# 17ai/eventql

Measured on AMD Instinct MI355X. Metric: rows/sec scanned+aggregated, 1e9-row 4-col GROUP BY, higher is better.
Workload: dtype u64/f64; 1 GPU; config3; query=k, sum(v), count(1), sum(b) WHERE a>30000 AND b<30000 GROUP BY k, rows_per_gpu=1000000000, columns=4, encodings=UINT64_PLAIN/FLOAT_IEEE754, groups=1000, partitions=1, merge=none, groups_hint=given, float_sums=fast

## Files before the change

### eventql_amd/csrc/codegen.h

```cpp
#pragma once
#include <string>
#include <vector>
#include "cstable_format.h"
#include "plan_ir.h"

namespace evql {

struct ColAccess {
  enum Mode { PLAIN64 = 0, PLAIN32 = 1, BITPACKED = 2, SOA = 3, NARROW = 4, NARROW_F32 = 5 };
  std::string name;
  uint32_t stype = EVQL_T_NIL;
  Mode mode = PLAIN64;
  uint32_t bits = 0;
  bool has_tags = false;
  bool bool_normalize = false;
  bool from_uint_to_float = false;
  bool string_hash = false;
  bool string_bytes = false;
  bool packed = false;
  bool dict_code = false;
  int layout_index = -1;
};

struct StateWord {
// ... 2 lines not shown

struct AggPlan {
  uint32_t fn = EVQL_AGG_NONE;
  ExprPtr arg;
  int first_word = 0;
  int nwords = 0;
  int distinct_index = -1;
  int exact_index = -1;
  bool narrow_arg = false;
};

static const int kMaxExactSums = 4;

static const int kMaxDistinct = 4;

static const int kMaxLits = 32;

static const uint64_t kZoneRows = 2048;
static const int kMaxZoneConjuncts = 4;

struct ZoneConjunct {
  int col = -1;
  uint32_t op = 0;
  uint64_t lit = 0;
};

enum KeyMode {
  KEY_NONE = 0,
  KEY_EXACT = 1,
  KEY_HASHED = 2
};

struct KernelPlan {
  std::vector<ColAccess> cols;
  ExprPtr where;
  std::vector<ExprPtr> group;
  std::vector<AggPlan> aggs;
  std::vector<StateWord> states;
  KeyMode key_mode = KEY_NONE;
  bool need_first_row = false;
  bool has_row_filter = false;
  int n_distinct = 0;
  int n_exact = 0;
  bool has_ident2() const { return key_mode == KEY_HASHED; }
  int first_row_word() const { return 1 + (has_ident2() ? 1 : 0); }
  int words_per_slot() const { return state_word_base() + int(states.size()); }
  int state_word_base() const { return first_row_word() + (need_first_row ? 1 : 0); }
  int block = 256;
  int unroll = 4;
  int lds_slots = 0;
  int lane_cache = 1;
  bool prefetch = false;
  bool prefetch_allowed = false;
  bool partitioned = false;
  int part_bits = 12;
  bool part_fused = false;
  bool narrow_ident = false;
  bool narrow_first_row = false;
  bool where_rows_kernel = false;
  bool bare_scan = false;
  std::vector<ExprPtr> scan_out;
  std::vector<bool> scan_out_nullable;
  std::vector<uint64_t> lit_pool;
  std::vector<ZoneConjunct> zone_conjuncts;
  int tile_rows() const { return block * 2 * unroll; }
};

void choose_launch_shape(KernelPlan* kp, uint64_t hint);
uint64_t lds_table_max_slots(const KernelPlan& kp);
extern const uint64_t kPartitionAboveSlots;
bool partitioned_path_possible(const KernelPlan& kp);

bool expr_prints_zero_check(const ExprPtr& e);

std::string generate_kernel_source(KernelPlan* kp);
int partition_tuple_u32_words(const KernelPlan& kp);

const char* device_library_source();

}
```

### eventql_amd/csrc/codegen_kernels.inc

```

namespace {

struct UpdWord {
  int word;
  int op;
  int tslot = -1;
  const char* constant = nullptr;
  bool narrow = false;
  int toff = -1;
};

struct Gen {
  const KernelPlan& kp;
  std::ostringstream s;
  const int NC, NW, S, W, SB;
  const bool grouped;
  std::vector<UpdWord> updw;

  explicit Gen(const KernelPlan& p)
      : kp(p), NC(int(p.cols.size())), NW(int(p.states.size())), S(p.lds_slots),
        W(p.words_per_slot()), SB(p.state_word_base()), grouped(p.key_mode != KEY_NONE) {
    for (const auto& a : kp.aggs) {
      switch (a.fn) {
        case EVQL_AGG_COUNT:
// ... 91 lines not shown
    char b[96];
    snprintf(b, sizeof(b), "A.gtab[(u64) %s * EVQL_WORDS + %d]", slot.c_str(), w);
    return b;
  }

  void prologue() {
    s << "// generated by eventql_amd codegen\n";
    s << "#define EVQL_BLOCK " << kp.block << "\n";
    s << "#define EVQL_UNROLL " << kp.unroll << "\n";
    s << "#define EVQL_TILE_ROWS " << kp.tile_rows() << "\n";
    s << "#define EVQL_LDS_SLOTS " << S << "\n";
    s << "#define EVQL_LSTRIDE " << (S + 2) << "\n";
    s << "#define EVQL_WORDS " << W << "\n";
    s << "#define EVQL_NSTATE " << NW << "\n";
    s << "#define EVQL_NUPD " << (U() > 0 ? U() : 1) << "\n";
    s << "#define EVQL_LCACHE " << kp.lane_cache << "\n";
    s << "#define EVQL_TUPLE_U32 " << tuple_u32 << "\n";
    s << "#define EVQL_TIF " << (tuple_u32 <= 10 ? 4 : 2) << "\n\n";
    s << "struct EvqlRowOut {\n  bool live;\n  bool knull;\n  u64 ident;\n  u64 ident2;\n"
         "  u64 ub[EVQL_NUPD];\n  bool uc[EVQL_NUPD];\n};\n\n";
  }

  template <typename Body>
  size_t row_function(size_t lit_base, Body body) {
    const std::string before = s.str();
    s.str("");
    Emitter em;
    em.lit_base = lit_base;
    em.pool = &pool;
    em.cols = &kp.cols;
    body(em);
    const std::string fn = s.str();
    s.str("");
    s << before;
    if (em.uses_strfn && !strfn_emitted) {
      s << strfn_library_source();
      strfn_emitted = true;
    }
    for (size_t i = 0; i < em.string_literals.size(); ++i) {
      const std::string& l = em.string_literals[i];
      s << "__device__ const u8 evql_slit" << (lit_base + i) << "[" << (l.empty() ? 1 : l.size())
        << "] = {";
      for (size_t k = 0; k < l.size(); ++k) s << (k ? "," : "") << unsigned((unsigned char) l[k]);
      if (l.empty()) s << "0";
      s << "};\n";
    }
    s << fn;
    return em.string_literals.size();
  }

  bool strfn_emitted = false;
  size_t n_literals = 0;
  std::vector<uint64_t> pool;
  void eval_row() {
    n_literals = row_function(0, [&](Emitter& em) { eval_row_body(em); });
  }

  void col_decls() {
    for (int i = 0; i < NC; ++i) {
      const ColAccess& c = kp.cols[i];
      s << "  const " << ctype(c.stype) << " c" << i << " = ";
      if (c.stype == EVQL_T_FLOAT64) {
        s << (c.from_uint_to_float ? "(double) r" : "evql_as_f64(r") << i
          << (c.from_uint_to_float ? "" : ")") << ";\n";
      } else if (c.stype == EVQL_T_BOOL) {
        s << "(r" << i << " != 0);\n";
      } else if (c.stype == EVQL_T_INT64) {
        s << "(i64) r" << i << ";\n";
      } else {
        s << "r" << i << ";\n";
      }
      s << "  (void) c" << i << "; (void) g" << i << ";\n";
    }
  }

  void eval_row_body(Emitter& em) {
    s << "__device__ __forceinline__ void evql_eval_row(const EvqlArgs& A, const u64 row, "
         "const bool valid";
    for (int i = 0; i < NC; ++i) s << ", const u64 r" << i << ", const u32 g" << i;
    s << ", EvqlRowOut& o) {\n";
    s << "  bool live = valid;\n";
    if (kp.has_row_filter) {
      s << "  live = live && evql_row_filter(A.row_filter, A.row_filter_len, row);\n";
    }
    col_decls();
    em.ind = "    ";
    if (kp.where) {
      s << "  if (live) {\n";
      Val p = em.emit(kp.where);
      s << em.o.str();
      em.o.str("");
      s << "    live = " << p.v << ";\n  }\n";
    }
    s << "  o.live = live;\n  o.knull = false;\n  o.ident = 0;\n  o.ident2 = 0;\n";
    for (int i = 0; i < U(); ++i) {
      s << "  o.ub[" << i << "] = evql_op_identity<" << op_name(updw[i].op) << ">(); o.uc[" << i
        << "] = false;\n";
    }
    s << "  if (live) {\n";
    if (kp.key_mode == KEY_EXACT) {
      Val k = em.emit(kp.group[0]);
      s << em.o.str();
      em.o.str("");
      s << "    o.ident = " << Emitter::as_bits(k) << ";\n";
      s << "    o.knull = (" << k.g << " & 1u) != 0;\n";
    } else if (kp.key_mode == KEY_HASHED) {
      s << "    u64 ident = EVQL_IDENT_SEED1, ident2 = EVQL_IDENT_SEED2;\n";
      for (const auto& g : kp.group) {
        Val k = em.emit(g);
        s << em.o.str();
        em.o.str("");
        s << "    evql_ident_add(ident, ident2, " << Emitter::as_bits(k) << ", " << k.g << ");\n";
      }
      s << "    o.ident = evql_ident_word(ident);\n";
      s << "    o.ident2 = evql_ident_word(ident2);\n";
    }
    int ui = 0;
    auto push = [&](const std::string& bits, const std::string& cond) {
      if (cond.empty()) {
        s << "    o.ub[" << ui << "] = " << bits << "; o.uc[" << ui << "] = true;\n";
      } else {
        s << "    o.uc[" << ui << "] = " << cond << ";\n";
        s << "    if (o.uc[" << ui << "]) o.ub[" << ui << "] = " << bits << ";\n";
      }
      ++ui;
    };
    for (const auto& a : kp.aggs) {
      Val v{"0", "0u", EVQL_T_NIL};
      if (a.arg) {
        v = em.emit(a.arg);
        s << em.o.str();
        em.o.str("");
      }
      const std::string notnull = "((" + v.g + " & 1u) == 0)";
      switch (a.fn) {
        case EVQL_AGG_COUNT:
          push("1ull", "");
          break;
        case EVQL_AGG_SUM_UINT64:
        case EVQL_AGG_SUM_INT64:
          push(Emitter::as_bits(v), "");
          break;
        case EVQL_AGG_SUM_FLOAT64:
          if (a.exact_index >= 0) {
            s << "    u64 fxh" << a.exact_index << ", fxl" << a.exact_index << ";\n";
            s << "    evql_fix(A, " << a.exact_index << ", " << v.v << ", fxh" << a.exact_index
              << ", fxl" << a.exact_index << ");\n";
            push("fxh" + std::to_string(a.exact_index), "");
            push("fxl" + std::to_string(a.exact_index), "");
          } else {
            push(Emitter::as_bits(v), "");
          }
          break;
        case EVQL_AGG_COUNT_DISTINCT_UINT64: {
          const char* flags = kp.key_mode == KEY_HASHED ? "o.ident2"
                              : (kp.key_mode == KEY_EXACT ? "(o.knull ? 1ull : 0ull)" : "0ull");
          char b[64];
          snprintf(b, sizeof(b), "evql_pairset_insert(A, %d, o.ident, ", a.distinct_index);
          push(std::string(b) + Emitter::as_bits(v) + ", " + flags + ", " +
                   (kp.key_mode == KEY_HASHED ? "false" : "true") + ")",
               "");
          break;
        }
        case EVQL_AGG_MEAN_UINT64:
        case EVQL_AGG_MEAN_INT64:
        case EVQL_AGG_MEAN_FLOAT64: {
          std::string d = a.fn == EVQL_AGG_MEAN_FLOAT64 ? v.v : "((double) " + v.v + ")";
          push("evql_f64_bits(" + d + ")", notnull);
          push("1ull", notnull);
          break;
        }
        default: {
          const bool is_f = a.fn == EVQL_AGG_MIN_FLOAT64 || a.fn == EVQL_AGG_MAX_FLOAT64;
          const std::string ok = is_f ? "(" + notnull + " && (" + v.v + " == " + v.v + "))" : notnull;
          push(Emitter::as_bits(v), ok);
          push("1ull", ok);
        }
      }
    }
    s << "  }\n}\n\n";
  }

  void tile_loads(const char* ind, const std::vector<bool>* only = nullptr) {
    for (int i = 0; i < NC; ++i) {
      if (only && !(*only)[i]) continue;
      s << ind << "u64 x" << i << "[EVQL_UNROLL][2]; u32 y" << i << "[EVQL_UNROLL][2];\n";
    }
    s << "#pragma unroll\n" << ind << "for (int u = 0; u < EVQL_UNROLL; ++u) {\n";
    s << ind << "  const u64 r = base + ((u64) (u * EVQL_BLOCK) + tid) * 2;\n";
    for (int i = 0; i < NC; ++i) {
      if (only && !(*only)[i]) continue;
      const ColAccess& c = kp.cols[i];
      switch (c.mode) {
        case ColAccess::PLAIN64:
          s << ind << "  evql_plain64_x2(A.col[" << i << "].base, A.col[" << i << "].pages, r, x" << i << "[u][0], x"
            << i << "[u][1]);\n";
          break;
        case ColAccess::PLAIN32:
          s << ind << "  evql_plain32_x2(A.col[" << i << "].base, A.col[" << i << "].pages, r, x" << i << "[u][0], x"
            << i << "[u][1]);\n";
          break;
        case ColAccess::BITPACKED:
          s << ind << "  evql_bitpacked_x2<" << c.bits << ">(A.col[" << i << "].base, A.col[" << i << "].pages, r, x"
            << i << "[u][0], x" << i << "[u][1]);\n";
          break;
        case ColAccess::NARROW:
          s << ind << "  evql_bitpacked_x2<" << c.bits << ">(A.col[" << i << "].base, r, x" << i
            << "[u][0], x" << i << "[u][1]);\n";
          break;
        case ColAccess::NARROW_F32:
          s << ind << "  evql_f32_x2(A.col[" << i << "].base, r, x" << i << "[u][0], x" << i
            << "[u][1]);\n";
          break;
        case ColAccess::SOA:
          s << ind << "  evql_soa_x2(A.col[" << i << "].soa, r, x" << i << "[u][0], x" << i
            << "[u][1]);\n";
          break;
      }
      if (c.has_tags) {
        s << ind << "  { const unsigned short tt = *reinterpret_cast<const unsigned short*>(A.col["
          << i << "].tags + r); y" << i << "[u][0] = tt & 0xffu; y" << i << "[u][1] = tt >> 8; }\n";
      } else {
        s << ind << "  y" << i << "[u][0] = 0; y" << i << "[u][1] = 0;\n";
      }
    }
    s << ind << "}\n";
  }

  bool prunes() const { return !kp.zone_conjuncts.empty(); }
  bool zone_test = false;
  template <typename Loop>
  void tile_loop_twice(const char* ind, Loop emit_loop) {
    zone_test = false;
// ... 69 lines not shown
      s << ind << "u32 " << name << i << "[EVQL_UNROLL][" << raw_words(kp.cols[i]) << "]"
        << (zero ? " = {}" : "") << ";\n";
    }
  }
  void raw_tile_loads(const char* ind) {
    s << "#pragma unroll\n" << ind << "for (int u = 0; u < EVQL_UNROLL; ++u) {\n";
    s << ind << "  const u64 r = lbase + ((u64) (u * EVQL_BLOCK) + tid) * 2;\n";
    for (int i = 0; i < NC; ++i) {
      const ColAccess& c = kp.cols[i];
      const int hi = raw_words(c) - 1;
      if (c.mode == ColAccess::NARROW_F32) {
        s << ind << "  evql_f32_x2(A.col[" << i << "].base, r, n" << i << "[u][0], n" << i << "[u][" << hi
          << "]);\n";
      } else {
        s << ind << "  evql_bitpacked_x2<" << c.bits << ">(A.col[" << i << "].base, r, n" << i << "[u][0], n"
          << i << "[u][" << hi << "]);\n";
      }
    }
    s << ind << "}\n";
  }
  void raw_step_decode(const char* ind) {
    s << ind << "asm(\"\" : ";
    bool first = true;
    for (int i = 0; i < NC; ++i) {
      for (int w = 0; w < raw_words(kp.cols[i]); ++w) {
        s << (first ? "" : ", ") << "\"+v\"(c" << i << "[u][" << w << "])";
        first = false;
      }
    }
    s << ");\n";
    for (int i = 0; i < NC; ++i) {
      const ColAccess& c = kp.cols[i];
      const int hi = raw_words(c) - 1;
      s << ind << "u64 x" << i << "s[2]; ";
      if (c.mode == ColAccess::NARROW_F32) {
        s << "evql_f32_dec(c" << i << "[u][0], c" << i << "[u][" << hi << "], x" << i << "s[0], x" << i
          << "s[1]);\n";
      } else {
        s << "evql_narrow_dec<" << c.bits << ">(c" << i << "[u][0], c" << i << "[u][" << hi << "], x" << i
          << "s[0], x" << i << "s[1]);\n";
      }
    }
  }
  void raw_tile_copy(const char* ind) {
    s << "#pragma unroll\n" << ind << "for (int u = 0; u < EVQL_UNROLL; ++u) {\n" << ind << " ";
    for (int i = 0; i < NC; ++i) {
      for (int w = 0; w < raw_words(kp.cols[i]); ++w) {
        s << " c" << i << "[u][" << w << "] = n" << i << "[u][" << w << "];";
      }
    }
    s << "\n" << ind << "}\n";
  }

  bool probe_ahead() const { return grouped && S > 0 && !kp.has_ident2(); }
  void scan_step(const std::string& ind, bool step_local) {
    const char* in = ind.c_str();
    if (probe_ahead()) {
      s << in << "EvqlRowOut o0, o1;\n";
      for (int j = 0; j < 2; ++j) eval_call(in, j, nullptr, j ? "o1" : "o0", step_local);
      for (int j = 0; j < 2; ++j) {
        s << in << "const u64 k" << j << " = evql_lds_peek(&lds[(u32) o" << j
          << ".ident & (EVQL_LDS_SLOTS - 1)]);\n";
      }
      for (int j = 0; j < 2; ++j) {
        s << in << "evql_update(A, lds, acc, bypass, r + " << j << ", o" << j << ", k" << j << ");\n";
      }
    } else {
      s << in << "EvqlRowOut o;\n";
      for (int j = 0; j < 2; ++j) {
        eval_call(in, j, nullptr, "o", step_local);
        s << in << "evql_update(A, lds, acc, bypass, r + " << j << ", o);\n";
      }
    }
  }
  void prefetch_tile_loop() {
    s << "  u32 tile_no = 0;  // tiles evaluated\n";
    raw_tile_decls("  ", "c", false);
    s << "  bool have = false;\n  u64 tc = 0;\n";
    s << "  for (u64 t = blockIdx.x; have || t < A.ntiles; t += gridDim.x) {\n";
    s << "    const bool more = t < A.ntiles;\n";
    s << "    const u64 tl = more ? t : tc;\n";
    s << "    u32 st = 0;\n";
    s << "    if ((tile_no & 15u) == 0) st = __hip_atomic_load(&A.status[0], __ATOMIC_RELAXED, "
         "__HIP_MEMORY_SCOPE_AGENT);\n";
    s << "    const u64 lbase = (A.tile0 + tl) * (u64) EVQL_TILE_ROWS;\n";
    raw_tile_decls("    ", "n", false);
    raw_tile_loads("    ");
    s << "    __builtin_amdgcn_sched_barrier(0);\n";
    s << "    if (have) {\n";
    s << "      const bool bypass = evql_lds_peek32(reinterpret_cast<const u32*>(&lds[EVQL_WORDS * "
         "EVQL_LSTRIDE])) >= 4u * EVQL_BLOCK;\n";
    s << "      const u64 base = (A.tile0 + tc) * (u64) EVQL_TILE_ROWS;\n";
    tile_window("      ");
    s << "#pragma unroll\n      for (int u = 0; u < EVQL_UNROLL; ++u) {\n";
    s << "        const u64 r = base + ((u64) (u * EVQL_BLOCK) + tid) * 2;\n";
    raw_step_decode("        ");
    scan_step("        ", true);
    s << "      }\n      ++tile_no;\n    }\n";
    s << "    __builtin_amdgcn_sched_barrier(0);\n";
    raw_tile_copy("    ");
    s << "    asm volatile(\"\" : \"+v\"(st)";
    for (int i = 0; i < NC; ++i) {
      for (int w = 0; w < raw_words(kp.cols[i]); ++w) s << ", \"+v\"(c" << i << "[EVQL_UNROLL - 1][" << w << "])";
    }
    s << ");\n";
    s << "    tc = tl;\n    have = more;\n";
    s << "    if (__builtin_amdgcn_readfirstlane(st) & EVQL_ST_TABLE_FULL) break;\n";
    s << "  }\n";
  }
  void scan_kernel() {
    const char* ctr = kp.prefetch ? "u32" : "u64";
    s << "struct EvqlAcc {\n  " << ctr << " passed;\n  " << ctr << " spilled;\n";
    if (!grouped) s << "  u64 w[" << (NW > 0 ? NW : 1) << "];\n";
    if (!grouped && kp.need_first_row) s << "  u64 first;\n";
    if (grouped && S > 0) {
      s << "  int cs[EVQL_LCACHE];\n  u64 cfirst[EVQL_LCACHE];\n  u64 cw[EVQL_LCACHE][EVQL_NUPD];\n"
           "  u32 cv;\n";
    }
    s << "};\n\n";
    if (grouped && S > 0) {
      s << "template <int J>\n";
      s << "__device__ __forceinline__ void evql_flush_entry(u64* lds, EvqlAcc& acc) {\n";
      s << "  const int cs = acc.cs[J];\n";
      if (kp.need_first_row) {
        s << "  evql_atomic<EVQL_OP_MIN_U64>(&" << lds_word(kp.first_row_word(), "cs") << ", acc.cfirst[J]);\n";
        s << "  acc.cfirst[J] = 0xFFFFFFFFFFFFFFFFull;\n";
      }
      for (int i = 0; i < U(); ++i) {
        s << "  evql_atomic<" << op_name(updw[i].op) << ">(&" << lds_word(SB + updw[i].word, "cs")
          << ", acc.cw[J][" << i << "]);\n";
        s << "  acc.cw[J][" << i << "] = evql_op_identity<" << op_name(updw[i].op) << ">();\n";
      }
      s << "}\n";
      s << "__device__ __forceinline__ void evql_flush_private(u64* lds, EvqlAcc& acc) {\n";
      for (int j = 0; j < kp.lane_cache; ++j) {
        s << "  if (acc.cs[" << j << "] >= 0) { evql_flush_entry<" << j << ">(lds, acc); acc.cs[" << j
          << "] = -1; }\n";
      }
      s << "}\n\n";
    }

    s << "__device__ __forceinline__ void evql_update(const EvqlArgs& A, u64* lds, EvqlAcc& acc,\n"
         "                                            const bool bypass, const u64 row, "
         "const EvqlRowOut& o"
      << (probe_ahead() ? ", const u64 slot0" : "") << ") {\n";
    s << "  acc.passed += o.live ? 1 : 0;\n";
    if (!grouped) {
      if (kp.need_first_row) s << "  if (o.live && row < acc.first) acc.first = row;\n";
      for (int i = 0; i < U(); ++i) {
        s << "  if (o.uc[" << i << "]) acc.w[" << updw[i].word << "] = evql_combine<"
          << op_name(updw[i].op) << ">(acc.w[" << updw[i].word << "], o.ub[" << i << "]);\n";
      }
      s << "}\n\n";
    } else {
      auto updates = [&](bool global, const char* slot, const char* ind) {
        if (kp.need_first_row) {
          s << ind << "evql_atomic<EVQL_OP_MIN_U64>(&"
            << (global ? gtab_word(kp.first_row_word(), slot) : lds_word(kp.first_row_word(), slot))
            << ", row);\n";
        }
        for (int i = 0; i < U(); ++i) {
// ... 89 lines not shown
    }

    if (grouped && S > 0) {
      s << "__device__ __forceinline__ void evql_lds_init(u64* lds) {\n";
      s << "  if (threadIdx.x == 0) lds[EVQL_WORDS * EVQL_LSTRIDE] = 0;\n";
      s << "  for (u32 i = threadIdx.x; i < EVQL_LSTRIDE; i += blockDim.x) {\n";
      s << "    lds[i] = EVQL_EMPTY;\n";
      if (kp.has_ident2()) s << "    lds[1 * EVQL_LSTRIDE + i] = EVQL_EMPTY;\n";
      if (kp.need_first_row) {
        s << "    " << lds_word(kp.first_row_word(), "i") << " = 0xFFFFFFFFFFFFFFFFull;\n";
      }
      for (int w = 0; w < NW; ++w) {
        s << "    " << lds_word(SB + w, "i") << " = evql_op_identity<" << op_name(kp.states[w].op)
          << ">();\n";
      }
      s << "  }\n}\n\n";
      s << "template <bool EXCL>\n";
      s << "__device__ __forceinline__ void evql_lds_flush(const EvqlArgs& A, u64* lds) {\n";
      s << "  const bool excl = EXCL && evql_lds_peek32(reinterpret_cast<const u32*>(&lds[EVQL_WORDS * EVQL_LSTRIDE])) "
           "== 0;\n";
      s << "  for (u32 s = threadIdx.x; s < EVQL_LSTRIDE; s += blockDim.x) {\n";
      s << "    const u64 k = lds[s];\n    if (k == EVQL_EMPTY) continue;\n";
      s << "    i64 gs;\n";
      s << "    if (s == EVQL_LDS_SLOTS) gs = (i64) A.gcap;\n";
      s << "    else if (s == EVQL_LDS_SLOTS + 1) gs = (i64) A.gcap + 1;\n";
      if (kp.has_ident2()) {
        s << "    else gs = evql_gtab_find2(A.gtab, EVQL_WORDS, A.gcap, k, lds[EVQL_LSTRIDE + s], "
             "evql_mix64(k));\n";
      } else {
        s << "    else gs = evql_gtab_find(A.gtab, EVQL_WORDS, A.gcap, k, evql_mix64(k));\n";
      }
      s << "    if (gs < 0) { atomicOr(&A.status[0], EVQL_ST_TABLE_FULL); continue; }\n";
      s << "    if (s >= EVQL_LDS_SLOTS) A.gtab[(u64) gs * EVQL_WORDS] = 0;\n";
      s << "    if (excl) {\n";
      if (kp.need_first_row) {
        s << "      " << gtab_word(kp.first_row_word(), "gs") << " = " << lds_word(kp.first_row_word(), "s")
          << ";\n";
      }
      for (int w = 0; w < NW; ++w) {
        s << "      " << gtab_word(SB + w, "gs") << " = " << lds_word(SB + w, "s") << ";\n";
      }
      s << "      continue;\n    }\n";
      if (kp.need_first_row) {
        s << "    evql_atomic<EVQL_OP_MIN_U64>(&" << gtab_word(kp.first_row_word(), "gs") << ", "
          << lds_word(kp.first_row_word(), "s") << ");\n";
      }
      for (int w = 0; w < NW; ++w) {
        s << "    evql_atomic<" << op_name(kp.states[w].op) << ">(&" << gtab_word(SB + w, "gs") << ", "
          << lds_word(SB + w, "s") << ");\n";
      }
      s << "  }\n}\n\n";
    }

    s << "extern \"C\" __global__ void __launch_bounds__(EVQL_BLOCK) evql_scan_agg(const EvqlArgs A) {\n";
    s << "  const u32 tid = threadIdx.x;\n";
    if (grouped && S > 0) {
      s << "  __shared__ u64 lds[EVQL_WORDS * EVQL_LSTRIDE + 1];\n";
      s << "  evql_lds_init(lds);\n  __syncthreads();\n";
    } else {
      s << "  u64* lds = nullptr;\n";
    }
    s << "  EvqlAcc acc;\n  acc.passed = 0;\n  acc.spilled = 0;\n";
    if (grouped && S > 0) {
      s << "  acc.cv = 0;\n";
      for (int j = 0; j < kp.lane_cache; ++j) {
        s << "  acc.cs[" << j << "] = -1;\n  acc.cfirst[" << j << "] = 0xFFFFFFFFFFFFFFFFull;\n";
        for (int i = 0; i < U(); ++i) {
          s << "  acc.cw[" << j << "][" << i << "] = evql_op_identity<" << op_name(updw[i].op) << ">();\n";
        }
      }
    }
    if (!grouped) {
      for (int w = 0; w < NW; ++w) {
        s << "  acc.w[" << w << "] = evql_op_identity<" << op_name(kp.states[w].op) << ">();\n";
      }
      if (kp.need_first_row) s << "  acc.first = 0xFFFFFFFFFFFFFFFFull;\n";
    }
    zone_skip_decl("  ");
    window32 = grouped;
    tile_loop_twice("  ", [&] {
    if (kp.prefetch && !zone_test && grouped && S > 0) {
      prefetch_tile_loop();
      return;
    }
    s << "  u32 tile_no = 0;\n";
    s << "  for (u64 t = blockIdx.x; t < A.ntiles; t += gridDim.x, ++tile_no) {\n";
    zone_skip("    ", "");
    if (grouped) {
      s << "    if ((tile_no & 15u) == 0 && (__hip_atomic_load(&A.status[0], __ATOMIC_RELAXED, "
           "__HIP_MEMORY_SCOPE_AGENT) & EVQL_ST_TABLE_FULL)) break;\n";
    }
    if (grouped && S > 0) {
      s << "    const bool bypass = evql_lds_peek32(reinterpret_cast<const u32*>(&lds[EVQL_WORDS * EVQL_LSTRIDE])) "
           ">= 4u * EVQL_BLOCK;\n";
    } else {
      s << "    const bool bypass = false;\n";
    }
    s << "    const u64 base = (A.tile0 + t) * (u64) EVQL_TILE_ROWS;\n";
    tile_window("    ");
    tile_loads("    ");
    s << "#pragma unroll\n    for (int u = 0; u < EVQL_UNROLL; ++u) {\n";
    s << "      const u64 r = base + ((u64) (u * EVQL_BLOCK) + tid) * 2;\n";
    scan_step("      ", false);
    s << "    }\n  }\n";
    });
    window32 = true;

    zone_skip_flush("  ");
    s << "  {\n    const u64 p = evql_wave_reduce<EVQL_OP_ADD_U64>(" << (kp.prefetch ? "(u64) " : "") << "acc.passed);\n";
    s << "    if ((tid & 63u) == 0 && p) atomicAdd(&A.counters[0], p);\n";
// ... 610 lines not shown
```

### eventql_amd/csrc/evql_device.h

```cpp
#ifndef EVQL_DEVICE_H
#define EVQL_DEVICE_H

typedef unsigned long long u64;
typedef long long i64;
typedef unsigned int u32;
typedef unsigned char u8;

#define EVQL_EMPTY 0xFFFFFFFFFFFFFFFFull
#define EVQL_MAX_COLS 16
#define EVQL_MAX_LITS 32
#define EVQL_WAVE 64

#define EVQL_ST_DIV_BY_ZERO 1u
#define EVQL_ST_TABLE_FULL 2u
#define EVQL_ST_MOD_BY_ZERO 4u

struct EvqlColArg {
  const u64* pages;
  const u64* soa;
  const u8* tags;
  u64 npages;
  const u64* strpos;
  const u8* base;
};
// ... 308 lines not shown
#define EVQL_OP_MIN_F64 6
#define EVQL_OP_MAX_F64 7

template <int OP>
__device__ __forceinline__ u64 evql_op_identity() {
  switch (OP) {
    case EVQL_OP_MIN_U64: return 0xFFFFFFFFFFFFFFFFull;
    case EVQL_OP_MAX_U64: return 0ull;
    case EVQL_OP_MIN_I64: return 0x7FFFFFFFFFFFFFFFull;
    case EVQL_OP_MAX_I64: return 0x8000000000000000ull;
    case EVQL_OP_MIN_F64: return 0x7FF0000000000000ull;
    case EVQL_OP_MAX_F64: return 0xFFF0000000000000ull;
    default: return 0ull;
  }
}

template <int OP>
__device__ __forceinline__ u64 evql_combine(u64 a, u64 b) {
  switch (OP) {
    case EVQL_OP_ADD_U64: return a + b;
    case EVQL_OP_ADD_F64: return evql_f64_bits(evql_as_f64(a) + evql_as_f64(b));
    case EVQL_OP_MIN_U64: return a < b ? a : b;
    case EVQL_OP_MAX_U64: return a > b ? a : b;
    case EVQL_OP_MIN_I64: return (i64) a < (i64) b ? a : b;
    case EVQL_OP_MAX_I64: return (i64) a > (i64) b ? a : b;
    case EVQL_OP_MIN_F64: return evql_as_f64(b) < evql_as_f64(a) ? b : a;
    case EVQL_OP_MAX_F64: return evql_as_f64(b) > evql_as_f64(a) ? b : a;
  }
  return a;
}

template <int OP>
__device__ __forceinline__ void evql_atomic(u64* p, u64 v) {
  switch (OP) {
    case EVQL_OP_ADD_U64: atomicAdd(p, v); break;
    case EVQL_OP_ADD_F64: unsafeAtomicAdd(reinterpret_cast<double*>(p), evql_as_f64(v)); break;
    case EVQL_OP_MIN_U64: atomicMin(p, v); break;
    case EVQL_OP_MAX_U64: atomicMax(p, v); break;
    case EVQL_OP_MIN_I64: atomicMin(reinterpret_cast<i64*>(p), (i64) v); break;
    case EVQL_OP_MAX_I64: atomicMax(reinterpret_cast<i64*>(p), (i64) v); break;
    case EVQL_OP_MIN_F64: unsafeAtomicMin(reinterpret_cast<double*>(p), evql_as_f64(v)); break;
    case EVQL_OP_MAX_F64: unsafeAtomicMax(reinterpret_cast<double*>(p), evql_as_f64(v)); break;
  }
}


__device__ __forceinline__ u64 evql_lds_peek(const u64* p) {
  return __hip_atomic_load(p, __ATOMIC_RELAXED, __HIP_MEMORY_SCOPE_WORKGROUP);
}
__device__ __forceinline__ u32 evql_lds_peek32(const u32* p) {
  return __hip_atomic_load(p, __ATOMIC_RELAXED, __HIP_MEMORY_SCOPE_WORKGROUP);
}

template <int MAXP>
__device__ __forceinline__ int evql_lds_find_from(u64* keys, u32 mask, u64 ident, u32 h, u64 cur) {
  u32 s = (u32) ident & mask;
  {
    if (cur == ident) return (int) s;
    if (cur == EVQL_EMPTY) {
      u64 old = atomicCAS(&keys[s], EVQL_EMPTY, ident);
      if (old == EVQL_EMPTY || old == ident) return (int) s;
    }
  }
  s = h & mask;
#pragma unroll 1
  for (int probe = 0; probe < MAXP; ++probe) {
    u64 cur = evql_lds_peek(&keys[s]);
    if (cur == ident) return (int) s;
    if (cur == EVQL_EMPTY) {
      u64 old = atomicCAS(&keys[s], EVQL_EMPTY, ident);
      if (old == EVQL_EMPTY || old == ident) return (int) s;
    }
    s = (s + 1) & mask;
  }
  return -1;
}
template <int MAXP>
__device__ __forceinline__ int evql_lds_find(u64* keys, u32 mask, u64 ident, u32 h) {
  return evql_lds_find_from<MAXP>(keys, mask, ident, h, evql_lds_peek(&keys[(u32) ident & mask]));
}

#define EVQL_GTAB_MAX_PROBE 128
__device__ __forceinline__ i64 evql_gtab_find(u64* tab, u32 W, u64 cap, u64 ident, u64 h) {
  const u64 mask = cap - 1;
  u64 s = h & mask;
  const u64 maxp = cap < EVQL_GTAB_MAX_PROBE ? cap : EVQL_GTAB_MAX_PROBE;
#pragma unroll 1
  for (u64 probe = 0; probe < maxp; ++probe) {
    u64* key = tab + s * W;
    u64 cur = __hip_atomic_load(key, __ATOMIC_RELAXED, __HIP_MEMORY_SCOPE_AGENT);
    if (cur == ident) return (i64) s;
    if (cur == EVQL_EMPTY) {
      u64 old = atomicCAS(key, EVQL_EMPTY, ident);
      if (old == EVQL_EMPTY || old == ident) return (i64) s;
    }
    s = (s + 1) & mask;
  }
  return -1;
}

template <int MAXP>
__device__ __forceinline__ int evql_lds_find2(u64* keys, u64* keys2, u32 mask, u64 ident,
                                              u64 ident2, u32 h) {
  u32 s = (u32) ident & mask;
#pragma unroll 1
  for (int probe = 0; probe <= MAXP; ++probe) {
// ... 84 lines not shown
```

### eventql_amd/csrc/planner.cc

```cpp
#include <cstdlib>
#include <cstring>
#include "runtime.h"

namespace evql {

namespace {

ExprPtr inline_inputs(const ExprPtr& e, const std::vector<ExprPtr>& sub, std::string* err) {
  if (!e) return e;
  if (e->kind == Expr::INPUT) {
    if (e->input >= sub.size()) {
      *err = "invalid input index";
      return e;
    }
    return sub[e->input];
  }
  auto c = std::make_shared<Expr>(*e);
  for (auto& a : c->args) a = inline_inputs(a, sub, err);
  return c;
}

bool has_agg_get(const ExprPtr& e) {
  if (!e) return false;
  if (e->kind == Expr::AGG_GET) return true;
// ... 184 lines not shown
    const ExprPtr &c = e->args[k], &l = e->args[1 - k];
    if (c->kind == Expr::INPUT && l->kind == Expr::LITERAL && !l->lit_tag && unsigned_type(l->type)) ci = k;
  }
  if (ci < 0) return;
  const ExprPtr& c = e->args[ci];
  if (c->input >= cols.size() || !unsigned_type(c->type)) return;
  const ColAccess& ca = cols[c->input];
  if (ca.stype != c->type || ca.layout_index < 0) return;
  if (ca.from_uint_to_float || ca.bool_normalize || ca.string_hash || ca.has_tags) return;
  if (!zone_column_qualifies(layout.columns[ca.layout_index])) return;
  ZoneConjunct z;
  z.col = int(c->input);
  z.lit = e->args[1 - ci]->lit_bits;
  switch (e->family) {
    case EVQL_FAM_EQ: z.op = ZONE_EQ; break;
    case EVQL_FAM_LT: z.op = ci == 0 ? ZONE_LT : ZONE_GT; break;
    case EVQL_FAM_LTE: z.op = ci == 0 ? ZONE_LTE : ZONE_GTE; break;
    case EVQL_FAM_GT: z.op = ci == 0 ? ZONE_GT : ZONE_LT; break;
    case EVQL_FAM_GTE: z.op = ci == 0 ? ZONE_GTE : ZONE_LTE; break;
    default: return;
  }
  out->push_back(z);
}

int op_for_minmax(uint32_t fn) {
  switch (fn) {
    case EVQL_AGG_MIN_UINT64: return 2;
    case EVQL_AGG_MAX_UINT64: return 3;
    case EVQL_AGG_MIN_INT64: return 4;
    case EVQL_AGG_MAX_INT64: return 5;
    case EVQL_AGG_MIN_FLOAT64: return 6;
    case EVQL_AGG_MAX_FLOAT64: return 7;
  }
  return 0;
}

}

uint64_t lds_table_max_slots(const KernelPlan& kp) {
  const uint64_t W = uint64_t(kp.words_per_slot());
  uint64_t smax = 256;
  while ((smax * 2 + 2) * 8 * W <= 150 * 1024) smax <<= 1;
  return smax;
}

bool partitioned_path_possible(const KernelPlan& kp) {
  return kp.key_mode != KEY_NONE &&
         !(kp.key_mode == KEY_EXACT && expr_may_be_null(kp.group[0], kp.cols)) &&
         kp.n_distinct == 0;
}

const uint64_t kPartitionAboveSlots = 1;

void choose_launch_shape(KernelPlan* kpp, uint64_t hint) {
  KernelPlan& kp = *kpp;
  kp.block = 256;
  kp.partitioned = false;
  kp.lane_cache = 1;
  kp.prefetch = false;
  kp.unroll = kp.cols.size() <= 2 ? 8 : 4;
  {
    int upd = 0;
    for (const auto& a : kp.aggs) upd += a.nwords;
    int per_step = 0;
    for (const auto& c : kp.cols) per_step += c.has_tags ? 5 : 4;
    while (kp.unroll > 1 && 50 + per_step * kp.unroll + 4 * upd > 144) kp.unroll /= 2;
  }
  kp.lds_slots = 0;
  if (kp.key_mode == KEY_NONE) return;
  const uint64_t smax = lds_table_max_slots(kp);
  if (hint > kPartitionAboveSlots * smax && partitioned_path_possible(kp)) {
    kp.partitioned = true;
    kp.lds_slots = int(smax);
    kp.block = 1024;
    kp.part_bits = 8;
    while (kp.part_bits < 14 && (hint >> kp.part_bits) > smax / 2) ++kp.part_bits;
  } else if (hint > 8 * smax) {
    kp.lds_slots = 0;
    kp.block = 256;
  } else {
    uint64_t s = smax;
    if (hint != 0) {
      s = 1024;
      while (s < hint * 4) s <<= 1;
      if (s > smax) s = smax;
    }
    kp.lds_slots = int(s);
    kp.block = 1024;
    kp.lane_cache = (hint >= 2 && hint <= 4) ? 4 : 1;
    bool raw = kp.prefetch_allowed && kp.key_mode == KEY_EXACT && !kp.bare_scan &&
               kp.unroll == 4 && kp.cols.size() >= 3 && !kp.has_row_filter && kp.n_distinct == 0;
    for (const auto& c : kp.cols) {
      raw = raw && (c.mode == ColAccess::NARROW || c.mode == ColAccess::NARROW_F32) && c.packed &&
            !c.has_tags && (c.bits == 8 || c.bits == 16 || c.bits == 32);
    }
    kp.prefetch = raw;
  }
}

Status build_kernel_plan(const TableLayout& layout, const evql_plan_desc_t* plan,
                         evql_query* q, bool* unsupported) {
  *unsupported = false;
  KernelPlan& kp = q->kp;
  auto unsup = [&](const std::string& m) {
    *unsupported = true;
    return Status::error(EVQL_ENOTSUP, m);
  };

  const bool within = plan->scan_mode == EVQL_SCAN_NESTED_WITHIN_RECORD;
  const bool nested = plan->scan_mode == EVQL_SCAN_NESTED || within;
  if (plan->scan_mode != EVQL_SCAN_FLAT && !nested) return Status::error(EVQL_EARG, "bad scan mode");
  q->nested = nested;
  q->within_record = within;
  if (within && plan->where) return unsup("WHERE in a WITHIN RECORD scan is not lowered");
  if (within && plan->n_scan_select == 0) {
    return Status::error(EVQL_EARG, "WITHIN RECORD scan without a scan select list");
  }
  if (nested && (plan->row_begin || plan->row_end)) return unsup("row range on a nested scan");
  if (plan->n_scan_columns > EVQL_MAX_COLS_HOST) return unsup("too many scan columns");
  const bool bare = plan->n_select == 0 && plan->n_group == 0 && plan->n_scan_select > 0;
  if (plan->n_select == 0 && !bare) {
    return unsup("bare scans are not lowered (no GROUP BY / aggregate)");
  }
  if (bare) {
    if (plan->group_mode == EVQL_MODE_PARTIAL) {
      return Status::error(EVQL_EARG, "a bare scan has no partial form");
    }
    if (within) return unsup("WITHIN RECORD bare scans are not lowered");
    if (plan->n_scan_select > kMaxEmitCols) return unsup("too many output columns in a bare scan");
  }

  for (uint32_t i = 0; i < plan->n_scan_columns; ++i) {
    ColAccess c;
    c.name = plan->scan_columns[i];
    c.stype = plan->scan_column_types[i];
    const ColumnLayout* cl = nullptr;
    for (size_t k = 0; k < layout.columns.size(); ++k) {
      if (layout.columns[k].name == c.name) {
        cl = &layout.columns[k];
        c.layout_index = int(k);
      }
    }
    if (!cl) {
      return Status::error(EVQL_EARG, "column not found: " + c.name);
    }
    if (cl->rlevel_max > 0 && !nested) return unsup("repeated column in a flat scan: " + c.name);
    switch (c.stype) {
      case EVQL_T_NIL:
        return Status::error(EVQL_EARG, "illegal column type: NIL");
// ... 334 lines not shown
          return unsup("aggregate function not lowerable");
      }
      q->select_agg_index[i] = int(kp.aggs.size());
      kp.aggs.push_back(a);
      if (has_input(lp.call)) {
        kp.need_first_row = true;
        first_row_beyond_key = true;
      }
    } else {
      if (has_agg_get(lp.call)) return Status::error(EVQL_EARG, "malformed aggregate program");
      ExprPtr e = inline_inputs(lp.call, scan_out, &err);
      if (!err.empty()) return Status::error(EVQL_EARG, err);
      if (kp.key_mode == KEY_EXACT && expr_equal(e, kp.group[0])) {
        q->select_passthrough[i] = true;
      } else if (!has_input(e)) {
      } else {
        kp.need_first_row = true;
        if (!(kp.group.size() == 1 && expr_equal(e, kp.group[0]))) first_row_beyond_key = true;
      }
    }
  }
  if (int(kp.states.size()) > kMaxStateWords) return unsup("too many aggregate state words");
  q->n_update_words = 0;
  for (const auto& a : kp.aggs) q->n_update_words += a.fn == EVQL_AGG_COUNT ? 0 : a.nwords;
  if (plan->group_mode == EVQL_MODE_PARTIAL && kp.key_mode == KEY_HASHED) {
    kp.need_first_row = true;
  }

  kp.has_row_filter = plan->row_filter_bits != nullptr;

  q->dict_candidate = -1;
  if (!nested && kp.key_mode == KEY_HASHED && kp.group.size() == 1 && kp.n_distinct == 0 &&
      !first_row_beyond_key && kp.group[0]->kind == Expr::INPUT &&
      kp.group[0]->input < kp.cols.size() && kp.cols[kp.group[0]->input].string_hash) {
    const uint32_t ki = kp.group[0]->input;
    std::vector<uint32_t> used;
    if (kp.where) expr_inputs(kp.where, &used);
    for (const auto& a : kp.aggs) {
      if (a.arg) expr_inputs(a.arg, &used);
    }
    bool elsewhere = false;
    for (uint32_t u2 : used) elsewhere = elsewhere || u2 == ki;
    if (!elsewhere) q->dict_candidate = int(ki);
  }

  kp.zone_conjuncts.clear();
  const char* zm = getenv("EVQL_ZONE_MAPS");
  if (!nested && kp.where && !(zm && strcmp(zm, "0") == 0) && !expr_prints_zero_check(kp.where)) {
    collect_zone_conjuncts(kp.where, layout, kp.cols, &kp.zone_conjuncts);
  }

  const char* pf = getenv("EVQL_SCAN_PREFETCH");
  kp.prefetch_allowed = !nested && !(pf && strcmp(pf, "0") == 0);

  choose_launch_shape(&kp, plan->groups_hint);
  return Status();
}

}
```

### eventql_amd/csrc/query_run.cc

```cpp
#include <algorithm>
#include <cmath>
#include <cstring>
#include "runtime.h"

evql_query::~evql_query() {
  if (d_gtab) hipFree(d_gtab);
  if (d_status) hipFree(d_status);
  if (d_counters) hipFree(d_counters);
  if (d_small_rec) hipFree(d_small_rec);
  if (h_tail && tail_pool) {
    if (launched) hipDeviceSynchronize();
    tail_pool->give(h_tail);
  }
  for (auto* p : d_pairset) {
    if (p) hipFree(p);
  }
  for (auto* p : d_mset) {
    if (p) hipFree(p);
  }
  if (d_row_filter && row_filter_owned) hipFree(d_row_filter);
  for (auto* c : chain) delete c;
  if (d_part_counts) hipFree(d_part_counts);
  if (d_bucket_start) hipFree(d_bucket_start);
  if (d_tuples) hipFree(d_tuples);
// ... 28 lines not shown
    ia.counters = q->d_counters;
  }
  return launch_table_init(ia, s);
}

static const uint32_t kEagerMaxRecords = 4096;
static const uint64_t kEagerMaxSlots = 1u << 18;
uint32_t eager_tail_records(const evql_query* q) {
  const KernelPlan& kp = q->kp;
  if (q->eager_tail == evql_query::EAGER_OFF) return 0;
  if (q->keep_table) return 0;
  if (q->in_chain) return 0;
  if (kp.bare_scan) return 0;
  if (kp.partitioned) return 0;
  if (q->dict_key) return 0;
  if (kp.n_distinct > 0) return 0;
  if (kp.need_first_row) return 0;
  if (!q->order.empty() && q->has_limit) return 0;
  if (q->gcap > kEagerMaxSlots) return 0;
  const uint64_t rw = uint64_t(kp.words_per_slot()) + 1;
  const uint64_t fit = (kTailBlockBytes / 8 - kTailRecords) / rw;
  return uint32_t(std::min<uint64_t>(fit, kEagerMaxRecords));
}

static Status alloc_gtab(evql_query* q, uint64_t gcap) {
  if (q->d_gtab) {
    hipFree(q->d_gtab);
    q->d_gtab = nullptr;
  }
  q->gcap = gcap;
  const uint64_t stride = gcap + 8;
  HIP_TRY(hipMalloc(reinterpret_cast<void**>(&q->d_gtab),
                    stride * uint64_t(q->kp.words_per_slot()) * 8));
  return Status();
}

static Status compile_plan_kernels(evql_query* q) {
  evql_ctx* ctx = q->ctx;
  if (q->kp.partitioned) {
    Status stw = choose_tuple_widths(q);
    if (!stw.ok()) return stw;
    evql_table* t = q->table;
    const uint64_t nrows = q->nested ? q->nested_rows : t->layout.num_rows;
    const uint64_t begin = std::min(q->row_begin, nrows);
    const uint64_t end = q->row_end ? std::min(q->row_end, nrows) : nrows;
    q->kp.part_fused = false;
    const uint64_t tw = uint64_t(partition_tuple_u32_words(q->kp)) / 2;
    q->kp.part_fused = q->kp.part_bits > 8 && !q->part_fused_off &&
                       (end - begin) * tw * 8 <= (16ull << 30);
  }
  q->source = generate_kernel_source(&q->kp);
  Status st = compile_kernel(ctx, q->source, &q->module, true);
  if (!st.ok()) return st;
  if (q->kp.prefetch) {
    int sc = 0;
    if (q->module.fn &&
        hipFuncGetAttribute(&sc, HIP_FUNC_ATTRIBUTE_LOCAL_SIZE_BYTES, q->module.fn) == hipSuccess && sc != 0) {
      q->kp.prefetch = false;
      q->kp.prefetch_allowed = false;
      q->source = generate_kernel_source(&q->kp);
      st = compile_kernel(ctx, q->source, &q->module, true);
      if (!st.ok()) return st;
    }
  }
  while (q->kp.unroll > 1) {
    int scratch = 0;
    hipFunction_t fns[5] = {q->kp.partitioned ? nullptr : q->module.fn, q->module.fn_count,
                            q->module.fn_scatter, q->module.fn_scan_count, q->module.fn_scan_emit};
    for (hipFunction_t f : fns) {
      int sc = 0;
      if (f && hipFuncGetAttribute(&sc, HIP_FUNC_ATTRIBUTE_LOCAL_SIZE_BYTES, f) == hipSuccess) {
        scratch = std::max(scratch, sc);
      }
    }
    if (scratch == 0) break;
    q->kp.unroll /= 2;
    q->source = generate_kernel_source(&q->kp);
    st = compile_kernel(ctx, q->source, &q->module, true);
    if (!st.ok()) return st;
  }
  int per_cu = 1;
  hipError_t oe = hipModuleOccupancyMaxActiveBlocksPerMultiprocessor(
      &per_cu, q->kp.bare_scan ? q->module.fn_scan_emit : q->module.fn, q->kp.block, 0);
  if (oe != hipSuccess || per_cu < 1) per_cu = 1;
  if (per_cu > 8) per_cu = 8;
  q->grid = ctx->num_cus * per_cu;
  return Status();
}

Status query_prepare(evql_query* q) {
  evql_table* t = q->table;
  const LeafLevels* where_leaf = nullptr;
  const bool record_filter = q->nested && (q->d_row_filter || !q->row_filter_host.empty());
  if (q->within_record) {
    Status st = materialize_within_record(q);
    if (!st.ok()) return st;
  } else if (q->nested) {
    Status st;
    if (!q->nested_siblings) {
      st = materialize_nested(q, q->kp.cols, &q->nested_flat, &q->nested_rows,
                              q->nested_where_mixed || record_filter ? &where_leaf : nullptr,
                              &q->nested_strpos);
      if (!st.ok() && st.code == EVQL_ENOTSUP && !q->nested_where_mixed &&
          st.msg.find("different repeated groups") != std::string::npos) {
        q->nested_siblings = true;
      } else if (!st.ok()) {
// ... 764 lines not shown
```

Before: 535.8 billion rows/s.

## Compact filtered rows into per-wave LDS ring before aggregation

Splits row evaluation into a WHERE pass and a post pass. Rows that pass the filter are packed into a per-wave LDS ring buffer using ballot/mbcnt compaction. Full waves of 64 survivors are then drained through key extraction and the hash-table update. This avoids divergent lanes doing aggregation work when the filter is selective, at the cost of LDS space, packing overhead and extra register pressure. A fallback recompiles without staging if the kernel spills to scratch.

New measurement: 567.8 billion rows/s (median of 6 runs). 1.06x the previous value.

```diff
diff --git a/eventql_amd/csrc/codegen.h b/eventql_amd/csrc/codegen.h
--- a/eventql_amd/csrc/codegen.h
+++ b/eventql_amd/csrc/codegen.h
@@ -78,6 +78,8 @@
   int lane_cache = 1;
   bool prefetch = false;
   bool prefetch_allowed = false;
+  bool stage = false;
+  bool stage_allowed = false;
   bool partitioned = false;
   int part_bits = 12;
   bool part_fused = false;
@@ -92,6 +94,17 @@
   int tile_rows() const { return block * 2 * unroll; }
 };
 
+struct StageField {
+  int col = -1;
+  int bits = 0;
+  bool f32 = false;
+  int word = 0;
+  int shift = 0;
+};
+static const int kStageRing = 128;
+static const uint64_t kLdsBytes = 160 * 1024;
+int stage_tuple_layout(const KernelPlan& kp, std::vector<StageField>* fields);
+
 void choose_launch_shape(KernelPlan* kp, uint64_t hint);
 uint64_t lds_table_max_slots(const KernelPlan& kp);
 extern const uint64_t kPartitionAboveSlots;
diff --git a/eventql_amd/csrc/codegen_kernels.inc b/eventql_amd/csrc/codegen_kernels.inc
--- a/eventql_amd/csrc/codegen_kernels.inc
+++ b/eventql_amd/csrc/codegen_kernels.inc
@@ -167,8 +167,29 @@
   bool strfn_emitted = false;
   size_t n_literals = 0;
   std::vector<uint64_t> pool;
+  bool staged() const { return kp.stage && kp.prefetch; }
   void eval_row() {
-    n_literals = row_function(0, [&](Emitter& em) { eval_row_body(em); });
+    if (!staged()) {
+      n_literals = row_function(0, [&](Emitter& em) { eval_row_body(em); });
+      return;
+    }
+    n_literals = row_function(0, [&](Emitter& em) {
+      row_signature("bool", "evql_where_row", "valid", false);
+      where_part(em);
+      s << "  return live;\n}\n\n";
+    });
+    n_literals += row_function(n_literals, [&](Emitter& em) {
+      row_signature("void", "evql_eval_post", "live", true);
+      col_decls();
+      post_part(em);
+      s << "}\n\n";
+    });
+    row_signature("void", "evql_eval_row", "valid", true);
+    for (int pass = 0; pass < 2; ++pass) {
+      s << (pass ? "), " : "  evql_eval_post(A, row, evql_where_row(A, row, valid, ");
+      for (int i = 0; i < NC; ++i) s << (i ? ", " : "") << "r" << i << ", g" << i;
+    }
+    s << ", o);\n}\n\n";
   }
 
   void col_decls() {
@@ -189,11 +210,13 @@
     }
   }
 
-  void eval_row_body(Emitter& em) {
-    s << "__device__ __forceinline__ void evql_eval_row(const EvqlArgs& A, const u64 row, "
-         "const bool valid";
+  void row_signature(const char* ret, const char* name, const char* flag, bool out) {
+    s << "__device__ __forceinline__ " << ret << " " << name << "(const EvqlArgs& A, const u64 row, "
+         "const bool " << flag;
     for (int i = 0; i < NC; ++i) s << ", const u64 r" << i << ", const u32 g" << i;
-    s << ", EvqlRowOut& o) {\n";
+    s << (out ? ", EvqlRowOut& o) {\n" : ") {\n");
+  }
+  void where_part(Emitter& em) {
     s << "  bool live = valid;\n";
     if (kp.has_row_filter) {
       s << "  live = live && evql_row_filter(A.row_filter, A.row_filter_len, row);\n";
@@ -207,6 +230,15 @@
       em.o.str("");
       s << "    live = " << p.v << ";\n  }\n";
     }
+  }
+  void eval_row_body(Emitter& em) {
+    row_signature("void", "evql_eval_row", "valid", true);
+    where_part(em);
+    post_part(em);
+    s << "}\n\n";
+  }
+  void post_part(Emitter& em) {
+    em.ind = "    ";
     s << "  o.live = live;\n  o.knull = false;\n  o.ident = 0;\n  o.ident2 = 0;\n";
     for (int i = 0; i < U(); ++i) {
       s << "  o.ub[" << i << "] = evql_op_identity<" << op_name(updw[i].op) << ">(); o.uc[" << i
@@ -293,7 +325,7 @@
         }
       }
     }
-    s << "  }\n}\n\n";
+    s << "  }\n";
   }
 
   void tile_loads(const char* ind, const std::vector<bool>* only = nullptr) {
@@ -469,6 +501,77 @@
     s << "\n" << ind << "}\n";
   }
 
+  std::vector<StageField> sfields;
+  int stage_words = 0;
+  static std::string stage_raw_field(const StageField& f, int j) {
+    const std::string c = "c" + std::to_string(f.col) + "[u]";
+    if (f.bits == 32) return c + "[" + std::to_string(j) + "]";
+    const std::string m = f.bits == 16 ? "0xffffu" : "0xffu";
+    return "((" + c + "[0] >> " + std::to_string(f.bits * j) + ") & " + m + ")";
+  }
+  void stage_tuple_text() {
+    stage_words = stage_tuple_layout(kp, &sfields);
+    s << "struct alignas(" << (stage_words % 2 == 0 ? 8 : 4) << ") EvqlStaged { u32 w[" << stage_words
+      << "]; };\n";
+    s << "__device__ __forceinline__ EvqlStaged evql_stage_pack(";
+    for (size_t k = 0; k < sfields.size(); ++k) s << (k ? ", " : "") << "const u32 f" << k;
+    s << ") {\n  EvqlStaged t;\n";
+    for (int w = 0; w < stage_words; ++w) {
+      s << "  t.w[" << w << "] = ";
+      bool first = true;
+      for (size_t k = 0; k < sfields.size(); ++k) {
+        if (sfields[k].word != w) continue;
+        s << (first ? "" : " | ");
+        if (sfields[k].shift) s << "(f" << k << " << " << sfields[k].shift << ")";
+        else s << "f" << k;
+        first = false;
+      }
+      s << ";\n";
+    }
+    s << "  return t;\n}\n";
+    for (const StageField& f : sfields) {
+      s << "__device__ __forceinline__ u64 evql_stage_col" << f.col << "(const EvqlStaged& t) {\n";
+      if (f.f32) {
+        s << "  u64 v0, v1;\n  evql_f32_dec(t.w[" << f.word << "], t.w[" << f.word << "], v0, v1);\n  return v0;\n";
+      } else if (f.bits == 32) {
+        s << "  return (u64) evql_opaque(t.w[" << f.word << "]);\n";
+      } else {
+        s << "  return (u64) evql_opaque((t.w[" << f.word << "] >> " << f.shift << ") & 0xffffu);\n";
+      }
+      s << "}\n";
+    }
+    s << "\n";
+  }
+  void stage_drain_function() {
+    s << "__device__ __forceinline__ void evql_stage_drain(const EvqlArgs& A, u64* lds, const EvqlStaged* ring,\n"
+         "                                                 EvqlAcc& acc, const bool bypass, u32& head, "
+         "const u32 lane, const bool live) {\n";
+    s << "  const EvqlStaged t = evql_stage_take(ring, head, lane);\n";
+    s << "  EvqlRowOut o;\n  evql_eval_post(A, 0ull, live";
+    for (int i = 0; i < NC; ++i) {
+      bool in = false;
+      for (const StageField& f : sfields) in = in || f.col == i;
+      if (in) s << ", evql_stage_col" << i << "(t), 0u";
+      else s << ", 0ull, 0u";
+    }
+    s << ", o);\n";
+    s << "  const u64 k = evql_lds_peek(&lds[(u32) o.ident & (EVQL_LDS_SLOTS - 1)]);\n";
+    s << "  evql_update(A, lds, acc, bypass, 0ull, o, k);\n}\n\n";
+  }
+  void stage_step(const std::string& ind) {
+    const char* in = ind.c_str();
+    for (int j = 0; j < 2; ++j) {
+      s << in << "if (tail - head >= 64u) evql_stage_drain(A, lds, ring, acc, bypass, head, lane, true);\n";
+      s << in << "const bool l" << j << " = evql_where_row(A, r + " << j << ", wrel + (u32) (u * EVQL_BLOCK * 2 + "
+        << j << ") < wlen";
+      for (int i = 0; i < NC; ++i) s << ", x" << i << "s[" << j << "], 0u";
+      s << ");\n";
+      s << in << "evql_stage_put(ring, tail, l" << j << ", evql_stage_pack(";
+      for (size_t k = 0; k < sfields.size(); ++k) s << (k ? ", " : "") << stage_raw_field(sfields[k], j);
+      s << "));\n";
+    }
+  }
+
   bool probe_ahead() const { return grouped && S > 0 && !kp.has_ident2(); }
   void scan_step(const std::string& ind, bool step_local) {
     const char* in = ind.c_str();
@@ -494,6 +597,11 @@
     s << "  u32 tile_no = 0;  // tiles evaluated\n";
     raw_tile_decls("  ", "c", false);
     s << "  bool have = false;\n  u64 tc = 0;\n";
+    if (staged()) {
+      s << "  EvqlStaged* const ring = evql_stage_ring + (tid >> 6) * EVQL_STAGE_RING;\n";
+      s << "  const u32 lane = tid & 63u;\n";
+      s << "  u32 head = 0, tail = 0;  // tuples this wave has taken out of its ring / put into it\n";
+    }
     s << "  for (u64 t = blockIdx.x; have || t < A.ntiles; t += gridDim.x) {\n";
     s << "    const bool more = t < A.ntiles;\n";
     s << "    const u64 tl = more ? t : tc;\n";
@@ -512,7 +620,8 @@
     s << "#pragma unroll\n      for (int u = 0; u < EVQL_UNROLL; ++u) {\n";
     s << "        const u64 r = base + ((u64) (u * EVQL_BLOCK) + tid) * 2;\n";
     raw_step_decode("        ");
-    scan_step("        ", true);
+    if (staged()) stage_step("        ");
+    else scan_step("        ", true);
     s << "      }\n      ++tile_no;\n    }\n";
     s << "    __builtin_amdgcn_sched_barrier(0);\n";
     raw_tile_copy("    ");
@@ -524,6 +633,15 @@
     s << "    tc = tl;\n    have = more;\n";
     s << "    if (__builtin_amdgcn_readfirstlane(st) & EVQL_ST_TABLE_FULL) break;\n";
     s << "  }\n";
+    if (staged()) {
+      s << "  {\n";
+      s << "    const bool bypass = evql_lds_peek32(reinterpret_cast<const u32*>(&lds[EVQL_WORDS * "
+           "EVQL_LSTRIDE])) >= 4u * EVQL_BLOCK;\n";
+      s << "    if (tail - head >= 64u) evql_stage_drain(A, lds, ring, acc, bypass, head, lane, true);\n";
+      s << "    const u32 left = tail - head;\n";
+      s << "    if (left) evql_stage_drain(A, lds, ring, acc, bypass, head, lane, lane < left);\n";
+      s << "  }\n";
+    }
   }
   void scan_kernel() {
     const char* ctr = kp.prefetch ? "u32" : "u64";
@@ -719,10 +837,16 @@
       s << "  }\n}\n\n";
     }
 
+    if (staged()) {
+      stage_tuple_text();
+      stage_drain_function();
+    }
+
     s << "extern \"C\" __global__ void __launch_bounds__(EVQL_BLOCK) evql_scan_agg(const EvqlArgs A) {\n";
     s << "  const u32 tid = threadIdx.x;\n";
     if (grouped && S > 0) {
       s << "  __shared__ u64 lds[EVQL_WORDS * EVQL_LSTRIDE + 1];\n";
+      if (staged()) s << "  __shared__ EvqlStaged evql_stage_ring[(EVQL_BLOCK / 64) * EVQL_STAGE_RING];\n";
       s << "  evql_lds_init(lds);\n  __syncthreads();\n";
     } else {
       s << "  u64* lds = nullptr;\n";
diff --git a/eventql_amd/csrc/evql_device.h b/eventql_amd/csrc/evql_device.h
--- a/eventql_amd/csrc/evql_device.h
+++ b/eventql_amd/csrc/evql_device.h
@@ -384,6 +384,23 @@
   return __hip_atomic_load(p, __ATOMIC_RELAXED, __HIP_MEMORY_SCOPE_WORKGROUP);
 }
 
+#define EVQL_STAGE_RING 128u
+template <typename T>
+__device__ __forceinline__ void evql_stage_put(T* ring, u32& tail, const bool live, const T& t) {
+  const u64 m = __builtin_amdgcn_ballot_w64(live);
+  const u32 below = __builtin_amdgcn_mbcnt_hi((u32) (m >> 32), __builtin_amdgcn_mbcnt_lo((u32) m, 0u));
+  if (live) ring[(tail + below) & (EVQL_STAGE_RING - 1u)] = t;
+  tail += (u32) __builtin_popcountll(m);
+}
+template <typename T>
+__device__ __forceinline__ T evql_stage_take(const T* ring, u32& head, const u32 lane) {
+  __builtin_amdgcn_fence(__ATOMIC_RELEASE, "wavefront");
+  __builtin_amdgcn_wave_barrier();
+  const T t = ring[(head + lane) & (EVQL_STAGE_RING - 1u)];
+  head += 64u;
+  return t;
+}
+
 template <int MAXP>
 __device__ __forceinline__ int evql_lds_find_from(u64* keys, u32 mask, u64 ident, u32 h, u64 cur) {
   u32 s = (u32) ident & mask;
diff --git a/eventql_amd/csrc/planner.cc b/eventql_amd/csrc/planner.cc
--- a/eventql_amd/csrc/planner.cc
+++ b/eventql_amd/csrc/planner.cc
@@ -260,12 +260,47 @@
 
 const uint64_t kPartitionAboveSlots = 1;
 
+int stage_tuple_layout(const KernelPlan& kp, std::vector<StageField>* fields) {
+  std::vector<uint32_t> used;
+  for (const auto& g : kp.group) expr_inputs(g, &used);
+  for (const auto& a : kp.aggs) {
+    if (a.arg) expr_inputs(a.arg, &used);
+  }
+  std::vector<bool> staged(kp.cols.size(), false);
+  for (uint32_t u : used) {
+    if (u < kp.cols.size()) staged[u] = true;
+  }
+  if (fields) fields->clear();
+  int halves = 0, words = 0;
+  for (int pass = 0; pass < 2; ++pass) {
+    for (size_t i = 0; i < kp.cols.size(); ++i) {
+      const ColAccess& c = kp.cols[i];
+      if (!staged[i] || (c.bits == 32) != (pass == 1)) continue;
+      StageField f;
+      f.col = int(i);
+      f.bits = int(c.bits);
+      f.f32 = c.mode == ColAccess::NARROW_F32;
+      if (pass == 0) {
+        f.word = halves / 2;
+        f.shift = 16 * (halves % 2);
+        ++halves;
+        words = (halves + 1) / 2;
+      } else {
+        f.word = words++;
+      }
+      if (fields) fields->push_back(f);
+    }
+  }
+  return words;
+}
+
 void choose_launch_shape(KernelPlan* kpp, uint64_t hint) {
   KernelPlan& kp = *kpp;
   kp.block = 256;
   kp.partitioned = false;
   kp.lane_cache = 1;
   kp.prefetch = false;
+  kp.stage = false;
   kp.unroll = kp.cols.size() <= 2 ? 8 : 4;
   {
     int upd = 0;
@@ -303,6 +338,13 @@
             !c.has_tags && (c.bits == 8 || c.bits == 16 || c.bits == 32);
     }
     kp.prefetch = raw;
+    if (raw && kp.stage_allowed && kp.where && !expr_always_true(kp.where) && !kp.need_first_row &&
+        !kp.has_ident2()) {
+      const uint64_t table = (uint64_t(kp.words_per_slot()) * (s + 2) + 1) * 8;
+      const uint64_t words = uint64_t(stage_tuple_layout(kp, nullptr));
+      const uint64_t ring = uint64_t(kp.block / 64) * kStageRing * 4 * words;
+      kp.stage = words >= 1 && table + ring <= kLdsBytes;
+    }
   }
 }
 
@@ -743,6 +785,8 @@
 
   const char* pf = getenv("EVQL_SCAN_PREFETCH");
   kp.prefetch_allowed = !nested && !(pf && strcmp(pf, "0") == 0);
+  const char* sg = getenv("EVQL_SCAN_STAGE");
+  kp.stage_allowed = kp.prefetch_allowed && !(sg && strcmp(sg, "0") == 0);
 
   choose_launch_shape(&kp, plan->groups_hint);
   return Status();
diff --git a/eventql_amd/csrc/query_run.cc b/eventql_amd/csrc/query_run.cc
--- a/eventql_amd/csrc/query_run.cc
+++ b/eventql_amd/csrc/query_run.cc
@@ -104,6 +104,17 @@
   q->source = generate_kernel_source(&q->kp);
   Status st = compile_kernel(ctx, q->source, &q->module, true);
   if (!st.ok()) return st;
+  if (q->kp.stage) {
+    int sc = 0;
+    if (q->module.fn &&
+        hipFuncGetAttribute(&sc, HIP_FUNC_ATTRIBUTE_LOCAL_SIZE_BYTES, q->module.fn) == hipSuccess && sc != 0) {
+      q->kp.stage = false;
+      q->kp.stage_allowed = false;
+      q->source = generate_kernel_source(&q->kp);
+      st = compile_kernel(ctx, q->source, &q->module, true);
+      if (!st.ok()) return st;
+    }
+  }
   if (q->kp.prefetch) {
     int sc = 0;
     if (q->module.fn &&
```
